# lh3/ropebwt2

Hardware: AMD Instinct MI355X
Metric: Gsymbols/s inserted (wall-clock), bit-identical .fmd (higher is better)
Workload: dtype u8; 1 GPU; configs[1]: 100000000 x 101 bp synthetic reads (splitmix64 seed 42), -bsR -m4g, 1 x MI355X; step = one -m batch (40844297/40844297/18311406 reads); 20 steps = 7 job(s) of 3 batches, each job on an empty index (the last job stops after batch 2); reads_per_job=100000000, symbols=69532236588, symbols_per_gpu=69532236588, parallelism=1 GPU, driver=single engine, counts_ok=True

## Files before the change

include/rb2_hip.h:

```cpp
#ifndef RB2_HIP_H_
#define RB2_HIP_H_

#include <stdint.h>

#ifdef __cplusplus
extern "C" {
#endif

typedef struct rb2_hip_s rb2_hip_t;

#define RB2_SO_IO   0
#define RB2_SO_RLO  1
#define RB2_SO_RCLO 2

typedef void (*rb2_hip_fatal_cb)(void *user, const char *message);
void rb2_hip_set_fatal_handler(rb2_hip_fatal_cb cb, void *user);

int rb2_hip_device_count(void);

rb2_hip_t *rb2_hip_create(int device, int sorting_order);
void rb2_hip_destroy(rb2_hip_t *h);
int  rb2_hip_sorting_order(const rb2_hip_t *h);
void rb2_hip_reset(rb2_hip_t *h);

// ... 71 lines not shown
void  rb2_hip_dev_free(rb2_hip_t *h, void *p);

void rb2_hip_synth_reads(rb2_hip_t *h, uint8_t *dst_dev, int64_t first_read, int64_t n_reads,
                         int read_len, uint64_t seed, int strand);
void rb2_hip_synth_reads_cov(rb2_hip_t *h, uint8_t *dst_dev, int64_t first_read, int64_t n_reads,
                             int read_len, uint64_t seed, int strand, int64_t genome_len);
void rb2_hip_synth_reads_skew(rb2_hip_t *h, uint8_t *dst_dev, int64_t first_read, int64_t n_reads,
                              int read_len, uint64_t seed, int strand, int64_t genome_len, int skew);

void rb2_hip_sync(rb2_hip_t *h);

void rb2_hip_sparse_stats(rb2_hip_t *h, int64_t out[4]);
void rb2_hip_layout_stats(rb2_hip_t *h, int64_t out[8]);
void rb2_hip_rewind_stats(rb2_hip_t *h, int64_t out[4]);
void rb2_hip_window_stats(rb2_hip_t *h, int64_t out[6]);

#define RB2_K_SYM      0
#define RB2_K_TSCAN    1
#define RB2_K_PREP     2
#define RB2_K_PART     3
#define RB2_K_MERGE    4
#define RB2_K_META     5
#define RB2_K_ADVANCE  6
#define RB2_K_INIT     7
#define RB2_K_RELAYOUT 8
#define RB2_K_SPLIT    9
#define RB2_K_COUNT    10
void rb2_hip_profile(rb2_hip_t *h, int enable);
void rb2_hip_profile_get(rb2_hip_t *h, int64_t launches[RB2_K_COUNT], double ms[RB2_K_COUNT],
                         int64_t units[RB2_K_COUNT], int reset);
// ... 9 lines not shown
```

ropebwt2_amd/csrc/rb2_device.h:

```cpp
#pragma once
#include <hip/hip_runtime.h>
#include <stddef.h>
#include <stdint.h>

namespace rb2 {

constexpr int SBITS  = 3;
constexpr int GSYM   = 64;
constexpr int LEAFG  = 16;
constexpr int LEAFW  = SBITS * LEAFG;
constexpr int LEAF   = GSYM * LEAFG;
constexpr int LEAF_SH = 10;
constexpr int SB     = 32;
constexpr int LEAFB  = LEAFW * 8;
#ifndef RB2_GPL
#define RB2_GPL 1
#endif
constexpr int GPL    = RB2_GPL;
constexpr int WPL    = 64 * GPL / LEAFG;
constexpr int WIN    = WPL * LEAF;
constexpr int STILE  = 512;
constexpr int MW     = 4;
constexpr int SCHUNK = 1024;
constexpr int ZBLOCK = 16384;
// ... 46 lines not shown
	uint64_t n0;
	uint64_t len;
	uint32_t ne[2];
	uint32_t wstride;
	uint32_t overflow;
	uint32_t sbfull;
	uint32_t nsplit2[2];
	uint64_t nsplit_total;
	RopeDesc relay_old[NR];
	uint32_t own[NR + 1];
	uint64_t sdest[NR][6];
	uint64_t pdst[NR][6];
	uint32_t pdev[NR][6];
	uint32_t wcnt[16 * 32];
	unsigned long long wfmt[4];
};
constexpr int GCN = NR * 6 + 2;
constexpr int WLC = 16;
constexpr int WLS = 32;

constexpr int NE_RING = 32;
struct Mailbox {
	volatile uint32_t void_round;
	volatile uint32_t respread;
	volatile uint32_t progress;
	uint32_t pad0;
	volatile unsigned long long hmax;
	uint64_t pad1;
	volatile unsigned long long hne;
	uint64_t pad2[3];
	volatile uint32_t ne[NE_RING][2];
// ... 415 lines not shown
```

ropebwt2_amd/csrc/rb2_engine.hip:

```cpp
#include <hip/hip_runtime.h>
#include <cstdio>
#include <cstdlib>
#include <cstring>
#include <climits>
#include <vector>
#include <algorithm>
#include <chrono>
#include <mutex>
#include <thread>
#include <condition_variable>
#include "rb2_hip.h"
#include "rb2_kernels.h"
#include "rb2_query.h"

using namespace rb2;

static rb2_hip_fatal_cb g_fatal_cb = nullptr;
static void *g_fatal_user = nullptr;
#include <cstdarg>
#include <atomic>
#include <mutex>
struct RankFail { std::atomic<int> failed{0}; std::mutex mu; char msg[1024]; };
static thread_local RankFail *t_rank_fail = nullptr;
struct RankAbort {};
// ... 170 lines not shown
	DevBuf<uint64_t> L[2], U[2], W[2], START, SIZE, INS_E, zblk;
	bool pos32 = false, want_pos32 = false;
	int pos_mode = getenv("RB2_POS") ? atoi(getenv("RB2_POS")) : 0;
	uint64_t pos_m0 = 0;
	DevBuf<uint16_t> RKREL;
	DevBuf<uint64_t> RKOLD;
	DevBuf<uint32_t> SPL;
	uint32_t split_epoch = 0;
	bool want_respread = false;
	int64_t n_respread = 0;
	DevBuf<uint64_t> qbuf;
	DevBuf<QTab> qtab;
	DevBuf<uint8_t> qbytes; DevBuf<int64_t> qin, qout;
	uint64_t sp_nsb = 0;
	DevBuf<LeafDesc> LD;
	DevBuf<uint8_t> A[2], INS_A, sbuf;
	DevBuf<uint8_t> sbuf2; hipStream_t st_copy = nullptr; const uint8_t *pf_host = nullptr; size_t pf_done = 0; std::mutex pf_mu;
	bool pf_busy = false; std::condition_variable pf_cv;
	static constexpr int UP_T = 6, UP_NB = 2; static constexpr size_t UP_CH = 8u << 20;
	uint8_t *up_pin[UP_T][UP_NB] = {}; hipStream_t up_st[UP_T] = {}; hipEvent_t up_ev[UP_T][UP_NB] = {}; bool up_init = false;
	DevBuf<TileRec> trec; DevBuf<TileScan> tsc; DevBuf<TileFix> tfix; DevBuf<ChunkPart> cpart;
	DevBuf<SbTot> sbtot;
	uint64_t *d_tmp = nullptr;
	int prof = 0;
	std::vector<ProfRec> recs;
	std::vector<hipEvent_t> evpool;
	int64_t p_launch[RB2_K_COUNT]; double p_ms[RB2_K_COUNT]; int64_t p_units[RB2_K_COUNT];
	int debug = 0;
	int cur_round = -1;
	uint64_t *gcnt = nullptr;
// ... 144 lines not shown
		h->START.ensure(m + 1);
		hipLaunchKernelGGL(k_write_starts, dim3(nzb), dim3(256), 0, st, s, len, h->zblk.p, h->START.p);
	}
	ensure_strings(h, m);
	B.nst_ub = cdiv(m, STILE) + NR;
	B.nsc = cdiv(B.nst_ub, SCHUNK);
	uint64_t n_tot = 0;
	for (int b = 0; b < NR; ++b) n_tot += h->h_rope[b].n;
	const uint64_t leaves_ub = (n_tot + len) / LEAF + NR * (SB + 1);
	if (!h->sparse) {
		h->pool[h->pside].ensure(leaves_ub, true, st);
		h->pool[h->pside ^ 1].ensure(leaves_ub, false, st);
	}
	if (!h->sparse) h->sbtot.ensure(leaves_ub / SB + 1);
	h->LD.ensure(std::max<uint64_t>(leaves_ub + NR + 16, m + 64 + (uint64_t)(NR + WLC + 1) * STILE / 2));
	B.s = s; B.len = len; B.m = m; B.n_tot = n_tot; B.nsb_ub = leaves_ub / SB + 1; B.cur = 0;
	{ uint64_t n0 = 0; for (int b = 0; b < NR; ++b) n0 += h->h_rope[b].cnt[0]; B.known_ae = B.known_ae0 = !is_srt || n0 == 0; }
	{
		uint64_t mx = 0;
		for (int b = 0; b < NR; ++b) mx = std::max<uint64_t>(mx, h->h_rope[b].n);
		h->pos_m0 = mx;
		h->pos32 = h->want_pos32 && h->pos_mode != 64 && mx + 2 * m < POS32_LIMIT;
		h->want_pos32 = false;
		h->mb_h->hmax = 0;
		h->mb_h->progress = 0;
	}
	{
		Scope sc(h, RB2_K_INIT, 0);
		hipLaunchKernelGGL(k_batch_setup, dim3(1), dim3(1), 0, st, h->ctl, h->side, m, len, is_srt);
		with_pos(h, B, [&](const auto &S) { using P = std::remove_pointer_t<decltype(S.L)>;
// ... 58 lines not shown
	hipStream_t st = h->st;
	const int sd = h->side;
	const int64_t units = (int64_t)B.m;
	h->cur_round = (int)r;
	const TileRecs trs = { (uint32_t*)h->trec.p, (uint32_t)(h->trec.cap & ~(size_t)3) };
	tl_slow(h, "start of round_counts");
	const bool one_launch_tail = B.nst_ub < (unsigned)h->ts_max;
	if (!spec) require_verdicts_seen(h, r, "counting phase without spec of round");
	SplitArgs sp; memset(&sp, 0, sizeof(sp));
	if (spec) {
	  sp.ctl = h->ctl; sp.pool = h->pool[h->pside].view(); sp.SPL = h->SPL.p; sp.spl_cap = split_cap(h); sp.epoch = h->split_epoch;
	  sp.mb = h->mb_d; sp.nsplitb = 64;
	  sp.round1 = (uint32_t)r;
	  sp.scan2 = (h->dir_ride && !one_launch_tail) ? sp.pool.sbbase : (SbBase*)nullptr;
	}
	SbBase *scan2_tail = (spec && h->dir_ride && one_launch_tail) ? h->pool[h->pside].view().sbbase : (SbBase*)nullptr;
	{ Scope sc(h, RB2_K_SYM, units);
	  with_pos(h, B, [&](const auto &S) { using P = std::remove_pointer_t<decltype(S.L)>;
	    if (spec) {
	      hipLaunchKernelGGL((k_sym<false, P, true>), dim3((unsigned)rank_share(h, B.nst_ub) + sp.nsplitb + (sp.scan2 ? 1u : 0u)), dim3(256), 0, st, h->ctl, sd, (int)(r & 1), S, trs, sp);
	    } else
	    RB2_LAUNCH_STRIDE(h, (k_sym<true, P>), (k_sym<false, P>), dim3(grid8((unsigned)rank_share(h, B.nst_ub))), dim3(256), 0, st, h->ctl, sd, (int)(r & 1), S, trs, sp); }); }
	tl_slow(h, "k_sym");
	if (spec && !lazy_round(h, spec)) HIPCHK(hipEventRecord(h->ev_flag, st));
	if (one_launch_tail) {
	  Scope sc(h, RB2_K_TSCAN, units);
	  const int do_setup = h->nranks == 1;
	  const unsigned grid = (unsigned)std::max(1, std::min<int>(TSB, h->ts_blocks)) + (scan2_tail ? 7u : 0u);
	  hipLaunchKernelGGL((h->sparse ? k_tscan_setup<true> : k_tscan_setup<false>), dim3(grid), dim3(SCHUNK), 0, st, h->ctl, sd, (int)(r & 1), trs, h->tfix.p, h->gcnt, do_setup, (int)spec, (uint32_t)r, hmax_report(h), scan2_tail);
	  if (do_setup) mark_setup(h, B, r);
	} else
	{ Scope sc(h, RB2_K_TSCAN, units);
	  hipLaunchKernelGGL(k_tscan1, dim3(B.nsc), dim3(SCHUNK), 0, st, h->ctl, sd, trs, h->cpart.p);
	  if (B.nsc <= (unsigned)h->ts_fold) hipLaunchKernelGGL(k_tscan3<true>, dim3(B.nsc), dim3(SCHUNK), 0, st, h->ctl, sd, trs, h->cpart.p, h->tsc.p);
	  else {
	    hipLaunchKernelGGL(k_tscan2, dim3(1), dim3(SCHUNK), 0, st, h->ctl, sd, h->cpart.p);
	    hipLaunchKernelGGL(k_tscan3<false>, dim3(B.nsc), dim3(SCHUNK), 0, st, h->ctl, sd, trs, h->cpart.p, h->tsc.p);
// ... 28 lines not shown
	hipStream_t st = h->st;
	const int sd = h->side;
	const int64_t units = (int64_t)B.m;
	PoolView oldp = h->pool[h->pside].view(), newp = h->pool[h->pside ^ 1].view();
	const uint64_t n_new_ub = B.n_tot + std::min<uint64_t>(B.len, (r + 1) * B.m);
	const unsigned nlf = cdiv(n_new_ub, WIN) + NR;
	const unsigned wg = cdiv(B.n_tot + rank_share(h, std::min<uint64_t>(B.len, (r + 1) * B.m)), WIN) + NR;
	if ((uint64_t)nlf * 64 >= (1ull << 32)) { rb2_fatal("[rb2_hip] the index is too large for one k_merge launch (%llu symbols: a launch is capped at 2^32 threads)\n", (unsigned long long)n_new_ub); }
	if (!setup_done(h, B, r, false))
	{ Scope sc(h, RB2_K_TSCAN, 0);
	  hipLaunchKernelGGL(k_setup<false>, dim3(1), dim3(64), 0, st, h->ctl, sd, h->gcnt, (int)(r & 1), (uint32_t)r, hmax_report(h), (int)(h->push[0] != nullptr)); }
	with_pos(h, B, [&](const auto &S) { using P = std::remove_pointer_t<decltype(S.L)>;
	launch_prep<false>(h, B, r, oldp, S);
	tl_slow(h, "k_prep");
	{ Scope sc(h, RB2_K_PART, units);
	  RB2_LAUNCH_STRIDE(h, (k_part<true, P>), (k_part<false, P>), dim3(cdiv(wg + NR, 255)), dim3(256), 0, st, h->ctl, sd, S.INS_E, h->LD.p, h->pool_compact ? (const uint8_t*)oldp.xh : (const uint8_t*)nullptr); }
	tl_slow(h, "k_part");
	{ Scope sc(h, RB2_K_MERGE, units);
	  RB2_LAUNCH_STRIDE(h, (k_merge<true, P>), (k_merge<false, P>), dim3(grid8(cdiv(wg, MMW))), dim3(64 * MMW), 0, st, h->ctl, h->LD.p, oldp, newp, S.INS_E, S.INS_A, S.RKREL, (int)compact_out | (h->compact_stats ? 2 : 0), (int)(r & 1)); }
	tl_slow(h, "k_merge");
	{ Scope sc(h, RB2_K_META, units);
	  build_directory(h, sd ^ 1, h->pside ^ 1, std::min<uint64_t>(B.nsb_ub, n_new_ub / (LEAF * SB) + NR + 1), false, false, (uint64_t)wg * WPL / SB + NR + 1); }
	tl_slow(h, "directory");
	launch_advance<false>(h, B, r, newp, S, send, ScanRide{ nullptr, 0u });
	});
	tl_slow(h, "k_advance");
	if (!B.known_ae && !send && h->nranks == 1) ne_snapshot(h, r);
	HIPCHK(hipGetLastError());
	tl_slow(h, "ne snapshot");
	h->side ^= 1; h->pside ^= 1; B.cur ^= 1;
	h->pool_compact = compact_out;
// ... 329 lines not shown
	if (getenv("RB2_SPARSE_MAXPEN")) h->sp_maxpen = atoi(getenv("RB2_SPARSE_MAXPEN"));
	if (h->trace) h->prof = 1;
	HIPCHK(hipStreamCreateWithFlags(&h->st, hipStreamNonBlocking));
	HIPCHK(hipMalloc((void**)&h->ctl, sizeof(Ctl)));
	HIPCHK(hipMalloc((void**)&h->d_tmp, 256));
	HIPCHK(hipMalloc((void**)&h->gcnt, GCN * 8));
	HIPCHK(hipHostMalloc((void**)&h->mb_h, sizeof(Mailbox), hipHostMallocDefault));
	memset(h->mb_h, 0, sizeof(Mailbox));
	HIPCHK(hipHostGetDevicePointer((void**)&h->mb_d, h->mb_h, 0));
	HIPCHK(hipEventCreateWithFlags(&h->ev_flag, hipEventDisableTiming));
	if (getenv("RB2_DIR_RIDE")) h->dir_ride = atoi(getenv("RB2_DIR_RIDE"));
	if (getenv("RB2_TS_BLOCKS")) h->ts_blocks = atoi(getenv("RB2_TS_BLOCKS"));
	if (getenv("RB2_LAZY_VERDICT")) h->lazy_verdict = atoi(getenv("RB2_LAZY_VERDICT"));
	if (getenv("RB2_RUN_AHEAD")) h->run_ahead = std::max(1, atoi(getenv("RB2_RUN_AHEAD")));
	if (getenv("RB2_VERDICT_POLL")) h->verdict_poll = atoi(getenv("RB2_VERDICT_POLL"));
	{ Ctl *hc = (Ctl*)calloc(1, sizeof(Ctl)); for (int b = 0; b < NR; ++b) hc->own[b] = 1; HIPCHK(hipMemcpy(h->ctl, hc, sizeof(Ctl), hipMemcpyHostToDevice)); free(hc); }
	HIPCHK(hipMemsetAsync(h->d_tmp, 0, 256, h->st));
	memset(h->h_rope, 0, sizeof(h->h_rope));
	memset(h->p_launch, 0, sizeof(h->p_launch)); memset(h->p_ms, 0, sizeof(h->p_ms)); memset(h->p_units, 0, sizeof(h->p_units));
	h->pool[0].ensure(SB * 8, false, h->st); h->pool[1].ensure(SB * 8, false, h->st);
	HIPCHK(hipStreamSynchronize(h->st));
	return h;
}

void rb2_hip_destroy(rb2_hip_t *h)
{ finish_pending(h);
	if (!h) return;
	HIPCHK(hipSetDevice(h->dev));
	if (h->own_stream) HIPCHK(hipStreamSynchronize(h->st)); else HIPCHK(hipDeviceSynchronize());
	for (int i = 0; i < 2; ++i) { h->pool[i].release(); h->L[i].release(); h->U[i].release(); h->W[i].release(); }
	h->START.release(); h->SIZE.release(); h->INS_E.release(); h->RKREL.release(); h->RKOLD.release(); h->SPL.release(); h->qbuf.release(); h->zblk.release(); h->qtab.release(); h->qbytes.release(); h->qin.release(); h->qout.release();
	h->LD.release(); h->A[0].release(); h->A[1].release(); h->INS_A.release(); h->sbuf.release(); h->sbuf2.release();
	if (h->st_copy) HIPCHK(hipStreamDestroy(h->st_copy));
	h->trec.release(); h->tsc.release(); h->tfix.release(); h->cpart.release(); h->sbtot.release();
	for (auto e : h->evpool) hipEventDestroy(e);
	HIPCHK(hipHostFree(h->mb_h)); HIPCHK(hipEventDestroy(h->ev_flag));

	if (h->pair_d) { HIPCHK(hipFree(h->pair_d)); HIPCHK(hipHostFree(h->pair_h)); }
	HIPCHK(hipFree(h->ctl)); HIPCHK(hipFree(h->d_tmp)); HIPCHK(hipFree(h->gcnt)); h->xstage.release(); h->xnb.release(); h->xpack.release(); h->xoff.release();
	for (int i = 0; i < 2; ++i) if (h->xhost[i]) { HIPCHK(hipHostFree(h->xhost[i])); HIPCHK(hipHostFree(h->xtot[i])); HIPCHK(hipEventDestroy(h->xev[i])); }
	if (h->own_stream) HIPCHK(hipStreamDestroy(h->st));
	delete h;
}

int rb2_hip_sorting_order(const rb2_hip_t *h) { return h->so; }

void rb2_hip_reset(rb2_hip_t *h)
// ... 543 lines not shown
	rb2_hip_synth_reads_cov(h, dst_dev, first_read, n_reads, read_len, seed, strand, 0);
}

void rb2_hip_reserve(rb2_hip_t *h, int64_t batch_bytes, int64_t batch_strings, int64_t total_symbols)
{ finish_pending(h);
	HIPCHK(hipSetDevice(h->dev));
	if (batch_bytes > 0) h->zblk.ensure(cdiv((uint64_t)batch_bytes, ZBLOCK) + 2);
	if (batch_strings > 0) ensure_strings(h, (uint64_t)batch_strings);
	if (total_symbols > 0) {
		const uint64_t leaves = (uint64_t)total_symbols / LEAF + NR * (SB + 1);
		size_t fr = 0, tot = 0;
		if (hipMemGetInfo(&fr, &tot) == hipSuccess && 2.0 * leaves * (LEAFB + 2.0 * sizeof(LeafMeta) + 2.0) > 0.6 * (double)fr) return;
		h->pool[h->pside].ensure(leaves, true, h->st);
		h->pool[h->pside ^ 1].ensure(leaves, false, h->st);
		h->LD.ensure(leaves + NR + 16);
		if (!h->sparse) h->sbtot.ensure(leaves / SB + 1);
	}
}

void rb2_hip_sparse_stats(rb2_hip_t *h, int64_t out[4])
{ finish_pending(h);
	out[0] = h->n_relayout; out[1] = h->n_void; out[2] = h->n_sparse_rounds; out[3] = h->sparse ? 1 : 0;
}

void rb2_hip_layout_stats(rb2_hip_t *h, int64_t out[8])
{ finish_pending(h);
	uint64_t ns = 0;
	HIPCHK(hipSetDevice(h->dev));
	HIPCHK(hipMemcpyAsync(&ns, &h->ctl->nsplit_total, 8, hipMemcpyDeviceToHost, h->st));
	HIPCHK(hipStreamSynchronize(h->st));
// ... 4 lines not shown
void rb2_hip_rewind_stats(rb2_hip_t *h, int64_t out[4])
{ finish_pending(h);
	out[0] = h->n_rewind; out[1] = h->n_rewound; out[2] = h->rewind_max; out[3] = h->n_rewind_even;
}

void rb2_hip_window_stats(rb2_hip_t *h, int64_t out[6])
{ finish_pending(h);
	unsigned long long w[4] = {0, 0, 0, 0};
	HIPCHK(hipSetDevice(h->dev));
	HIPCHK(hipMemcpyAsync(w, &h->ctl->wfmt[0], sizeof(w), hipMemcpyDeviceToHost, h->st));
	HIPCHK(hipStreamSynchronize(h->st));
	for (int i = 0; i < 4; ++i) out[i] = (int64_t)w[i];
	out[4] = h->n_compact_rounds; out[5] = h->compact_stats ? 1 : 0;
}

void rb2_hip_sync(rb2_hip_t *h) { finish_pending(h); HIPCHK(hipSetDevice(h->dev)); HIPCHK(hipStreamSynchronize(h->st)); }

void rb2_hip_profile(rb2_hip_t *h, int enable) { finish_pending(h); h->prof = enable; }

void rb2_hip_profile_get(rb2_hip_t *h, int64_t launches[RB2_K_COUNT], double ms[RB2_K_COUNT], int64_t units[RB2_K_COUNT], int reset)
{ finish_pending(h);
	for (int k = 0; k < RB2_K_COUNT; ++k) { launches[k] = h->p_launch[k]; ms[k] = h->p_ms[k]; units[k] = h->p_units[k]; }
	if (reset) { memset(h->p_launch, 0, sizeof(h->p_launch)); memset(h->p_ms, 0, sizeof(h->p_ms)); memset(h->p_units, 0, sizeof(h->p_units)); }
}

const char *rb2_hip_kernel_name(int k)
{
	static const char *nm[RB2_K_COUNT] = {"k_sym", "k_tscan", "k_prep", "k_part", "k_merge", "k_meta", "k_advance", "k_init", "k_relayout", "k_split"};
	return (k >= 0 && k < RB2_K_COUNT) ? nm[k] : "?";
}
// ... 12 lines not shown
```

ropebwt2_amd/csrc/rb2_kernels.h:

```cpp
#pragma once
#include "rb2_device.h"

namespace rb2 {


__device__ __forceinline__ uint32_t zero_bytes(uint32_t x)
{
	const uint32_t t = ((x & 0x7f7f7f7fu) + 0x7f7f7f7fu) | x;
	return __popc(~t & 0x80808080u);
}

__device__ __forceinline__ void load64(const uint8_t *s, uint64_t len, uint64_t base, uint32_t w[16])
{
	if (base + 64 <= len) {
		const uint4 *p = (const uint4*)(s + base);
#pragma unroll
		for (int i = 0; i < 4; ++i) { uint4 v = p[i]; w[4*i] = v.x; w[4*i+1] = v.y; w[4*i+2] = v.z; w[4*i+3] = v.w; }
	} else {
#pragma unroll
		for (int i = 0; i < 16; ++i) {
			uint32_t x = 0;
			for (int k = 0; k < 4; ++k) {
				const uint64_t p = base + 4*i + k;
				x |= (uint32_t)(p < len ? s[p] : 0xffu) << (8*k);
// ... 162 lines not shown
__global__ __launch_bounds__(256) void k_widen(const uint32_t *src, uint64_t *dst, uint64_t n)
{
	const uint64_t i = (uint64_t)blockIdx.x * 256 + threadIdx.x;
	if (i < n) dst[i] = src[i];
}

__global__ void k_batch_setup(Ctl *ctl, int side, uint64_t m, uint64_t len, int is_srt)
{
	if (threadIdx.x || blockIdx.x) return;
	SegDesc &sg = ctl->seg[side];
	for (int b = 0; b < NR; ++b) { sg.start[b] = 0; sg.cnt[b] = 0; }
	sg.cnt[0] = ctl->own[0] ? m : 0;
	uint32_t t = 0;
	for (int b = 0; b < NR; ++b) { sg.tile0[b] = t; t += (uint32_t)((sg.cnt[b] + STILE - 1) / STILE); }
	sg.tile0[NR] = t; sg.tile0[NR + 1] = t;
	uint64_t n0 = 0;
	for (int b = 0; b < NR; ++b) n0 += ctl->rope[side][b].cnt[0];
	ctl->n0 = n0; ctl->n_strings = m; ctl->max_len = 0; ctl->len = len;
	ctl->ne[0] = (is_srt && n0) ? 1u : 0u;
	ctl->ne[1] = 0;
}


struct TileCtx { int b; uint64_t lt, base, segstart, segend; };

__device__ __forceinline__ bool tile_ctx(const SegDesc &sg, uint32_t tile, TileCtx &t)
{
	if (tile >= sg.tile0[NR]) return false;
	const int b = seg_of(sg.tile0, tile);
	t.b = b; t.lt = tile - sg.tile0[b];
	t.segstart = sg.start[b]; t.segend = sg.start[b] + sg.cnt[b];
	t.base = t.segstart + t.lt * STILE;
	return true;
}

struct SplitArgs { Ctl *ctl; PoolView pool; const uint32_t *SPL; uint32_t spl_cap, epoch; Mailbox *mb; uint32_t nsplitb;
	uint32_t round1;
	SbBase *scan2; };
template <int NT, int CT> __device__ __forceinline__ void sbscan2_lean(const Ctl *ctl, SbBase *base, uint64_t *s_w );
template <int NT, int CT> __device__ __forceinline__ void sbscan2_col(const Ctl *ctl, SbBase *base, uint64_t *s_w, const int col);
__device__ __forceinline__ void split_body(Ctl *ctl, const PoolView &pool, const uint32_t *SPL, uint32_t spl_cap, uint32_t epoch, Mailbox *mb,
		const uint32_t bidx, const uint32_t nblk, uint16_t (*s_row)[7][SB], uint32_t round1);
constexpr int32_t TILE_DONE = 0x10000;
constexpr int32_t TILE_SINGLE = 0x20000;
template <bool STRIDE, typename P = uint64_t, bool SPLIT = false> __global__ __launch_bounds__(256) void k_sym(const Ctl *ctl, int side, int par, StrArrays<P> S, TileRecs trec, SplitArgs sp)
{
	const P *L = S.L, *UU = S.U; P *INS_E = S.INS_E; uint8_t *INS_A = S.INS_A, *A = S.A;
	__shared__ uint64_t s_bal[8][6], s_head[8];
	__shared__ __align__(16) uint32_t s_ok[4];
	if (SPLIT) {
		__shared__ uint16_t s_row[MW][7][SB];
		if (blockIdx.x < sp.nsplitb) { split_body(sp.ctl, sp.pool, sp.SPL, sp.spl_cap, sp.epoch, sp.mb, blockIdx.x, sp.nsplitb, s_row, sp.round1); return; }
		if (sp.scan2 && blockIdx.x == sp.nsplitb) { __shared__ uint64_t s_w2[4]; sbscan2_lean<256, 2>(ctl, sp.scan2, s_w2); return; }
	}
	const bool ae = ctl->ne[par] == 0;
	const P *U = ae ? L : UU;
	for (uint32_t tile = (STRIDE || SPLIT) ? blockIdx.x - (SPLIT ? sp.nsplitb + (sp.scan2 ? 1u : 0u) : 0u) : xcd_item(); ; tile += gridDim.x) {
	if (STRIDE && tile != blockIdx.x) __syncthreads();
	TileCtx t;
	if (!tile_ctx(ctl->seg[side], tile, t)) return;
	const int ln = lane_id(), w = wave_id();
	const uint32_t nval = (uint32_t)min((uint64_t)STILE, t.segend - t.base);
	const uint8_t *Ab = A + t.base; const P *Ub = U + t.base;
	const bool first_tile = t.base == t.segstart;
	uint32_t av[2]; P uv[2], up[2], un = 0;
#pragma unroll
	for (int h = 0; h < 2; ++h) {
		const uint32_t x = (uint32_t)(h * 256) + threadIdx.x;
		RB2_UNDEFV(av[h]); RB2_UNDEFV(uv[h]); RB2_UNDEFV(up[h]);
		if (x < nval) { av[h] = Ab[x]; uv[h] = Ub[x]; up[h] = (x > 0 || !first_tile) ? Ub[(int32_t)x - 1] : (P)0; }
	}
	const bool last_thread = threadIdx.x == 255;
	const bool has_next = last_thread && t.base + STILE < t.segend;
	if (has_next) un = Ub[STILE];
	bool single = true;
	int sym2[2];
	uint8_t *Aw = A + t.base;
#pragma unroll
	for (int h = 0; h < 2; ++h) {
		const uint32_t x = (uint32_t)(h * 256) + threadIdx.x;
		int sym = 7; bool head = false;
		if (x < nval) {
			sym = (int)(av[h] & 7);
			head = (x == 0 && first_tile) || (uv[h] != up[h]);
			Aw[x] = (uint8_t)(sym | (head ? 0x80 : 0));
			single = single && head;
		}
		sym2[h] = sym;
		const int c = h * 4 + w;
// ... 11 lines not shown
	{ const uint64_t sm = ballot64(single); if (ln == 0) s_ok[w] = sm == ~0ull ? 1u : 0u; }
	__syncthreads();
	const uint4 okv = *(const uint4*)s_ok;
	const bool allsingle = (okv.x & okv.y & okv.z & okv.w) != 0;
	const bool fused = ae && allsingle;
	if (fused) {
		P *Eb = INS_E + t.base; uint8_t *Ib = INS_A + t.base;
		const P slot0 = (P)(t.lt * STILE);
#pragma unroll
		for (int h = 0; h < 2; ++h) {
			const uint32_t x = (uint32_t)(h * 256) + threadIdx.x;
			if (x >= nval) continue;
			Eb[x] = (P)(uv[h] - (slot0 + (P)x));
			Ib[x] = (uint8_t)sym2[h];
		}
	}
	if (threadIdx.x < 6) {
		const int s = threadIdx.x;
		uint32_t run = 0, fhpre = 0, lhpre = 0; int fh = -1, lh = -1;
		if (allsingle) {
#pragma unroll
			for (int c = 0; c < 8; ++c) run += __popcll(s_bal[c][s]);
			if (nval) { fh = 0; lh = (int)nval - 1; lhpre = run - (uint32_t)((s_bal[lh >> 6][s] >> (lh & 63)) & 1ull); }
		} else
		for (int c = 0; c < 8; ++c) {
			const uint64_t hm = s_head[c], bm = s_bal[c][s];
			if (hm) {
				const int f = __builtin_ctzll(hm), l = 63 - __builtin_clzll(hm);
				if (fh < 0) { fh = c * 64 + f; fhpre = run + __popcll(bm & lt_mask(f)); }
				lh = c * 64 + l; lhpre = run + __popcll(bm & lt_mask(l));
			}
// ... 193 lines not shown
		const uint64_t pinc = dpp_incl_add64(padded), winc = dpp_incl_add64(nwin);
		n.leaf0 = pinc - padded; n.sb0 = n.leaf0 / SB;
		if (ok) { ctl->rope[side ^ 1][r] = n; ctl->wf0[r] = winc - nwin; }
		if (r == 63) { ctl->wf0[NR] = winc; ctl->wf0[NR + 1] = winc; ctl->nsb_total = pinc / SB; }
	}
	uint64_t c2 = 0;
	if (ok && r != 0 && ctl->own[r]) {
		const int a = rope_sym(r), b = rope_prev(r);
		if (b == 0) c2 = gcnt[a];
		else for (int x = 0; x < 6; ++x) c2 += gcnt[rope_of(b, x) * 6 + a];
	}
	const uint64_t cinc = dpp_incl_add64(c2), st = cinc - c2;
	const uint32_t nt = (uint32_t)((c2 + STILE - 1) / STILE);
	const uint32_t tinc = dpp_incl_add(nt);
	if (ok) { ng.start[r] = st; ng.cnt[r] = c2; ng.tile0[r] = tinc - nt; }
	if (r == 63) { ng.tile0[NR] = tinc; ng.tile0[NR + 1] = tinc; }
	for (int a = 1; a < 6; ++a) {
		const int r2 = rope_of(a, rope_sym(rr));
		const uint64_t st2 = __shfl(st, r2);
		uint64_t before = 0;
		if (rope_sym(rr) != 0) for (int x = 0; x < rope_prev(rr); ++x) before += gcnt[rope_of(rope_sym(rr), x) * 6 + a];
		if (ok) ctl->dest[r][a] = st2 + before;
	}
	if (ok) ctl->dest[r][0] = 0;
}
template <bool SPARSE> __global__ __launch_bounds__(64) void k_setup(Ctl *ctl, int side, const uint64_t *gcnt, int par, uint32_t round, volatile unsigned long long *hmax, int keep_ne)
{
	if (blockIdx.x) return;
	setup_body<SPARSE>(ctl, side, gcnt, par, round, hmax, keep_ne != 0);
}
// ... 336 lines not shown
			prep_tile<AE, SPARSE, P>(t0 + k, ctl, side, par, is_comp, oldp, S);
			if (todo) __syncthreads();
		}
		return;
	}
	for (uint32_t tile = STRIDE ? blockIdx.x : xcd_item(); ; ) {
		if (!prep_tile<AE, SPARSE, P>(tile, ctl, side, par, is_comp, oldp, S)) return;
		if (!STRIDE) return;
		tile += gridDim.x;
		if (tile >= ctl->seg[side].tile0[NR]) return;
		__syncthreads();
	}
}


template <bool STRIDE, typename P = uint64_t> __global__ __launch_bounds__(256) void k_part(const Ctl *ctl, int side, const P *INS_E, LeafDesc *LD, const uint8_t *old_xh)
{
	__shared__ uint64_t s_wf0[NR + 1];
	__shared__ uint32_t s_q[256];
	if (threadIdx.x <= NR) s_wf0[threadIdx.x] = ctl->wf0[threadIdx.x];
	__syncthreads();
	for (uint64_t blk = blockIdx.x; blk * 255 < s_wf0[NR] + NR; blk += gridDim.x) {
	if (STRIDE && blk != blockIdx.x) __syncthreads();
	const uint64_t gid = blk * 255 + threadIdx.x;
	const bool ok = gid < s_wf0[NR] + NR;
	int b = 0; uint64_t j = 0; uint32_t q = 0;
	if (ok) {
		while (gid >= s_wf0[b+1] + b + 1) ++b;
		j = gid - s_wf0[b] - b;
		const SegDesc &sg = ctl->seg[side];
		const P *E = INS_E + sg.start[b];
		const uint64_t o = j * WIN;
		uint64_t lo = 0, hi = sg.cnt[b];
		while (lo < hi) {
			const uint64_t mid = (lo + hi) >> 1;
			if (E[mid] + mid >= o) hi = mid; else lo = mid + 1;
		}
		q = (uint32_t)lo;
	}
	s_q[threadIdx.x] = q;
	__syncthreads();
	if (!ok || threadIdx.x == 255 || j >= s_wf0[b+1] - s_wf0[b]) { if (!STRIDE) return; continue; }
	const RopeDesc &orp = ctl->rope[side][b], &nrp = ctl->rope[side ^ 1][b];
	const uint32_t q1 = s_q[threadIdx.x + 1];
	const uint64_t o0 = j * WIN, i0 = o0 - q;
	LeafDesc d;
	d.i0 = i0;
	d.ins0 = ctl->seg[side].start[b] + q;
	d.gl = nrp.leaf0 + j * WPL;
	d.oleaf0 = (uint32_t)orp.leaf0;
	const uint64_t ow = i0 >> 12, onw = (orp.nleaves + WPL - 1) / WPL;
	static_assert(WPL * LEAF == 4096, "a window is 4096 symbols");
	const uint8_t *xw = old_xh ? old_xh + orp.leaf0 / WPL : nullptr;
	const uint32_t h0 = ow < onw ? (xw ? (uint32_t)xw[ow] & 3u : 0u) : 1u;
	const uint32_t h1 = ow + 1 < onw ? (xw ? (uint32_t)xw[ow + 1] & 3u : 0u) : 1u;
	d.ni = (uint16_t)((uint32_t)(q1 - q) | h0 << 14);
	d.nvalid = (uint16_t)((uint32_t)min((uint64_t)WIN, nrp.n - o0) | h1 << 14);
	LD[s_wf0[b] + j] = d;
	if (!STRIDE) return;
// ... 972 lines not shown
```

ropebwt2_amd/hipbwt.py:

```python
import ctypes as C
import os

import numpy as np

from .build import lib_path

K_NAMES = ["k_sym", "k_tscan", "k_prep", "k_part", "k_merge", "k_meta", "k_advance", "k_init", "k_relayout", "k_split"]
_lib = None


def load_hip_lib():
    global _lib
    if _lib is not None:
        return _lib
    path = os.environ.get("RB2_HIP_LIB") or lib_path("librb2hip.so")
    if not os.path.exists(path):
        raise RuntimeError("%s missing: run `python -m ropebwt2_amd.build` (hipcc, gfx950) first" % path)
    L = C.CDLL(path)
    vp, i64, i32, u64 = C.c_void_p, C.c_int64, C.c_int, C.c_uint64
    sig = {
        "rb2_hip_device_count": (i32, []),
        "rb2_hip_set_fatal_handler": (None, [vp, vp]),
        "rb2_hip_create": (vp, [i32, i32]),
        "rb2_hip_destroy": (None, [vp]),
# ... 19 lines not shown
        "rb2_hip_extract": (i64, [vp, i64, vp, i64, vp, vp]),
        "rb2_hip_reserve": (None, [vp, i64, i64, i64]),
        "rb2_hip_num_subropes": (i32, []),
        "rb2_hip_memcpy": (None, [vp, vp, vp, i64, i32]),
        "rb2_hip_use_stream": (None, [vp, vp]),
        "rb2_hip_dev_alloc": (vp, [vp, i64]),
        "rb2_hip_dev_free": (None, [vp, vp]),
        "rb2_hip_synth_reads": (None, [vp, vp, i64, i64, i32, u64, i32]),
        "rb2_hip_synth_reads_cov": (None, [vp, vp, i64, i64, i32, u64, i32, i64]),
        "rb2_hip_synth_reads_skew": (None, [vp, vp, i64, i64, i32, u64, i32, i64, i32]),
        "rb2_hip_sync": (None, [vp]),
        "rb2_hip_sparse_stats": (None, [vp, vp]),
        "rb2_hip_layout_stats": (None, [vp, vp]),
        "rb2_hip_rewind_stats": (None, [vp, vp]),
        "rb2_hip_window_stats": (None, [vp, vp]),
        "rb2_hip_host_register": (C.c_int, [vp, C.c_int64]),
        "rb2_hip_host_unregister": (C.c_int, [vp]),
        "rb2_hip_profile": (None, [vp, i32]),
        "rb2_hip_profile_get": (None, [vp, vp, vp, vp, i32]),
        "rb2_hip_kernel_name": (C.c_char_p, [i32]),
        "rb2_hip_layout": (None, [vp, vp, vp]),
        "rb2_hip_multi_create": (vp, [i32, vp, i32, i32, vp]),
        "rb2_hip_multi_unique_id": (None, [vp]),
        "rb2_hip_multi_create_rank": (vp, [i32, i32, i32, vp, i32, vp]),
        "rb2_hip_multi_destroy": (None, [vp]),
        "rb2_hip_default_owners": (None, [i32, vp]),
        "rb2_hip_multi_nranks": (i32, [vp]),
        "rb2_hip_multi_transport": (i32, [vp]),
        "rb2_hip_multi_nlocal": (i32, [vp]),
        "rb2_hip_multi_engine": (vp, [vp, i32]),
# ... 21 lines not shown
            if os.environ.get("RB2_HIP_LIB"):
                continue
            raise
        f.restype = res
        f.argtypes = args
    _lib = L
    return L


ABI_SYMBOLS = [
    "rb2_hip_device_count", "rb2_hip_set_fatal_handler", "rb2_hip_create", "rb2_hip_destroy", "rb2_hip_sorting_order", "rb2_hip_reset",
    "rb2_hip_insert_multi", "rb2_hip_insert_multi_dev", "rb2_hip_set_lazy", "rb2_hip_wait", "rb2_hip_last_batch_counts", "rb2_hip_prefetch", "rb2_hip_mem_info", "rb2_hip_get_counts", "rb2_hip_rope_bytes",
    "rb2_hip_download_rope", "rb2_hip_stream_rope", "rb2_hip_load_ropes", "rb2_hip_rank1a", "rb2_hip_rank_batch", "rb2_hip_reserve",
    "rb2_hip_backward_search", "rb2_hip_backward_search_dev", "rb2_hip_extend", "rb2_hip_extract", "rb2_hip_dev_alloc",
    "rb2_hip_num_subropes", "rb2_hip_memcpy", "rb2_hip_use_stream",
    "rb2_hip_dev_free", "rb2_hip_synth_reads", "rb2_hip_synth_reads_cov", "rb2_hip_synth_reads_skew", "rb2_hip_sync", "rb2_hip_sparse_stats", "rb2_hip_layout_stats", "rb2_hip_rewind_stats", "rb2_hip_window_stats", "rb2_hip_host_register", "rb2_hip_host_unregister", "rb2_hip_profile",
    "rb2_hip_profile_get", "rb2_hip_kernel_name", "rb2_hip_layout",
    "rb2_hip_multi_create", "rb2_hip_multi_unique_id", "rb2_hip_multi_create_rank", "rb2_hip_multi_destroy", "rb2_hip_default_owners",
    "rb2_hip_multi_nranks", "rb2_hip_multi_transport", "rb2_hip_multi_nlocal", "rb2_hip_multi_engine", "rb2_hip_multi_insert_multi", "rb2_hip_multi_insert_multi_dev",
    "rb2_hip_multi_get_counts", "rb2_hip_multi_rope_bytes", "rb2_hip_multi_download_rope", "rb2_hip_multi_stream_rope",
    "rb2_hip_multi_load_ropes", "rb2_hip_multi_reserve", "rb2_hip_multi_rope_hash", "rb2_hip_rope_hash", "rb2_hip_multi_plan_host", "rb2_hip_multi_reset", "rb2_hip_multi_sync", "rb2_hip_multi_rank1a", "rb2_hip_multi_stats", "rb2_hip_multi_text_bytes",
]


_NT6 = np.full(256, 255, dtype=np.uint8)
for _i, _ch in enumerate("$ACGTN"):
    _NT6[ord(_ch)] = _NT6[ord(_ch.lower())] = _i


def encode_pattern(p):
    if isinstance(p, str):
# ... 192 lines not shown
        a = np.zeros(8, np.int64)
        self.L.rb2_hip_layout_stats(self.h, a.ctypes.data)
        return {"relayouts": int(a[0]), "void_rounds": int(a[1]), "sparse_rounds": int(a[2]), "sparse_now": bool(a[3]),
                "respreads": int(a[4]), "leaf_splits": int(a[5]), "grown_in_rounds": int(a[6]), "plain_handovers": int(a[7])}

    def rewind_stats(self):
        a = np.zeros(4, np.int64)
        self.L.rb2_hip_rewind_stats(self.h, a.ctypes.data)
        return {"rewinds": int(a[0]), "rounds_taken_back": int(a[1]), "deepest": int(a[2]), "even_depth": int(a[3])}

    def window_stats(self):
        a = np.zeros(6, np.int64)
        self.L.rb2_hip_window_stats(self.h, a.ctypes.data)
        return {"plain": int(a[0]), "compact0": int(a[1]), "compact1": int(a[2]), "compact2": int(a[3]), "compact_rounds": int(a[4]), "counted": bool(a[5])}

    def profile(self, on=True):
        self.L.rb2_hip_profile(self.h, int(on))

    def profile_get(self, reset=False):
        n = len(K_NAMES)
        la = np.zeros(n, np.int64)
        ms = np.zeros(n, np.float64)
        un = np.zeros(n, np.int64)
        self.L.rb2_hip_profile_get(self.h, la.ctypes.data, ms.ctypes.data, un.ctypes.data, 1 if reset else 0)
        return {K_NAMES[i]: {"launches": int(la[i]), "ms": float(ms[i]), "units": int(un[i])} for i in range(n)}

    @staticmethod
    def layout():
        L = load_hip_lib()
        a, b, c = C.c_int(), C.c_int(), C.c_int()
# ... 116 lines not shown
```

Baseline: 23.10 Gsymbols/s.

## Build window-to-insert lookup table in k_sym so k_part skips binary search

k_sym now scatters, for each insertion, its index into a per-window table QT, using per-rope window offsets that are precomputed in the segment setup and advance kernels. k_part then reads the window start indices straight from this table and no longer binary-searches INS_E per window, which also removes a shared-memory exchange and a barrier. The change adds scattered writes in k_sym, extra Ctl fields and a fallback flag (q_bad) that returns k_part to the binary search when runs are too long or the capacity is exceeded. A verify mode (2) counts mismatches for debugging.

```diff
diff --git a/include/rb2_hip.h b/include/rb2_hip.h
--- a/include/rb2_hip.h
+++ b/include/rb2_hip.h
@@ -109,6 +109,7 @@
 void rb2_hip_layout_stats(rb2_hip_t *h, int64_t out[8]);
 void rb2_hip_rewind_stats(rb2_hip_t *h, int64_t out[4]);
 void rb2_hip_window_stats(rb2_hip_t *h, int64_t out[6]);
+void rb2_hip_part_table_stats(rb2_hip_t *h, int64_t out[4]);
 
 #define RB2_K_SYM      0
 #define RB2_K_TSCAN    1
diff --git a/ropebwt2_amd/csrc/rb2_device.h b/ropebwt2_amd/csrc/rb2_device.h
--- a/ropebwt2_amd/csrc/rb2_device.h
+++ b/ropebwt2_amd/csrc/rb2_device.h
@@ -84,7 +84,13 @@
 	uint32_t pdev[NR][6];
 	uint32_t wcnt[16 * 32];
 	unsigned long long wfmt[4];
-};
+	uint32_t q_bad;
+	uint32_t q_rounds;
+	uint32_t q_mismatch;
+	uint32_t q_pad;
+	uint64_t q_wf0[2][NR + 1];
+};
+struct QArgs { uint32_t *Q; uint32_t cap, run, pad; };
 constexpr int GCN = NR * 6 + 2;
 constexpr int WLC = 16;
 constexpr int WLS = 32;
diff --git a/ropebwt2_amd/csrc/rb2_engine.hip b/ropebwt2_amd/csrc/rb2_engine.hip
--- a/ropebwt2_amd/csrc/rb2_engine.hip
+++ b/ropebwt2_amd/csrc/rb2_engine.hip
@@ -208,6 +208,9 @@
 	DevBuf<uint8_t> qbytes; DevBuf<int64_t> qin, qout;
 	uint64_t sp_nsb = 0;
 	DevBuf<LeafDesc> LD;
+	DevBuf<uint32_t> QT;
+	int part_table = 1;
+	uint32_t q_run = 0;
 	DevBuf<uint8_t> A[2], INS_A, sbuf;
 	DevBuf<uint8_t> sbuf2; hipStream_t st_copy = nullptr; const uint8_t *pf_host = nullptr; size_t pf_done = 0; std::mutex pf_mu;
 	bool pf_busy = false; std::condition_variable pf_cv;
@@ -382,6 +385,7 @@
 	}
 	if (!h->sparse) h->sbtot.ensure(leaves_ub / SB + 1);
 	h->LD.ensure(std::max<uint64_t>(leaves_ub + NR + 16, m + 64 + (uint64_t)(NR + WLC + 1) * STILE / 2));
+	if (h->nranks == 1 && h->part_table) h->QT.ensure(leaves_ub / WPL + NR + 16);
 	B.s = s; B.len = len; B.m = m; B.n_tot = n_tot; B.nsb_ub = leaves_ub / SB + 1; B.cur = 0;
 	{ uint64_t n0 = 0; for (int b = 0; b < NR; ++b) n0 += h->h_rope[b].cnt[0]; B.known_ae = B.known_ae0 = !is_srt || n0 == 0; }
 	{
@@ -470,13 +474,15 @@
 	  sp.round1 = (uint32_t)r;
 	  sp.scan2 = (h->dir_ride && !one_launch_tail) ? sp.pool.sbbase : (SbBase*)nullptr;
 	}
+	if (++h->q_run == 0) h->q_run = 1;
+	const QArgs qa = { (h->nranks == 1 && h->part_table) ? h->QT.p : (uint32_t*)nullptr, (uint32_t)std::min<size_t>(h->QT.cap, 0xffffffffu), h->q_run, 0u };
 	SbBase *scan2_tail = (spec && h->dir_ride && one_launch_tail) ? h->pool[h->pside].view().sbbase : (SbBase*)nullptr;
 	{ Scope sc(h, RB2_K_SYM, units);
 	  with_pos(h, B, [&](const auto &S) { using P = std::remove_pointer_t<decltype(S.L)>;
 	    if (spec) {
-	      hipLaunchKernelGGL((k_sym<false, P, true>), dim3((unsigned)rank_share(h, B.nst_ub) + sp.nsplitb + (sp.scan2 ? 1u : 0u)), dim3(256), 0, st, h->ctl, sd, (int)(r & 1), S, trs, sp);
+	      hipLaunchKernelGGL((k_sym<false, P, true>), dim3((unsigned)rank_share(h, B.nst_ub) + sp.nsplitb + (sp.scan2 ? 1u : 0u)), dim3(256), 0, st, h->ctl, sd, (int)(r & 1), S, trs, sp, qa);
 	    } else
-	    RB2_LAUNCH_STRIDE(h, (k_sym<true, P>), (k_sym<false, P>), dim3(grid8((unsigned)rank_share(h, B.nst_ub))), dim3(256), 0, st, h->ctl, sd, (int)(r & 1), S, trs, sp); }); }
+	    RB2_LAUNCH_STRIDE(h, (k_sym<true, P>), (k_sym<false, P>), dim3(grid8((unsigned)rank_share(h, B.nst_ub))), dim3(256), 0, st, h->ctl, sd, (int)(r & 1), S, trs, sp, qa); }); }
 	tl_slow(h, "k_sym");
 	if (spec && !lazy_round(h, spec)) HIPCHK(hipEventRecord(h->ev_flag, st));
 	if (one_launch_tail) {
@@ -535,7 +541,8 @@
 	launch_prep<false>(h, B, r, oldp, S);
 	tl_slow(h, "k_prep");
 	{ Scope sc(h, RB2_K_PART, units);
-	  RB2_LAUNCH_STRIDE(h, (k_part<true, P>), (k_part<false, P>), dim3(cdiv(wg + NR, 255)), dim3(256), 0, st, h->ctl, sd, S.INS_E, h->LD.p, h->pool_compact ? (const uint8_t*)oldp.xh : (const uint8_t*)nullptr); }
+	  RB2_LAUNCH_STRIDE(h, (k_part<true, P>), (k_part<false, P>), dim3(cdiv(wg + NR, 255)), dim3(256), 0, st, h->ctl, sd, S.INS_E, h->LD.p, h->pool_compact ? (const uint8_t*)oldp.xh : (const uint8_t*)nullptr,
+	    (const uint32_t*)h->QT.p, (uint32_t)std::min<size_t>(h->QT.cap, 0xffffffffu), h->q_run, h->nranks == 1 ? h->part_table : 0, (int)(r & 1)); }
 	tl_slow(h, "k_part");
 	{ Scope sc(h, RB2_K_MERGE, units);
 	  RB2_LAUNCH_STRIDE(h, (k_merge<true, P>), (k_merge<false, P>), dim3(grid8(cdiv(wg, MMW))), dim3(64 * MMW), 0, st, h->ctl, h->LD.p, oldp, newp, S.INS_E, S.INS_A, S.RKREL, (int)compact_out | (h->compact_stats ? 2 : 0), (int)(r & 1)); }
@@ -895,6 +902,7 @@
 	if (getenv("RB2_LAZY_VERDICT")) h->lazy_verdict = atoi(getenv("RB2_LAZY_VERDICT"));
 	if (getenv("RB2_RUN_AHEAD")) h->run_ahead = std::max(1, atoi(getenv("RB2_RUN_AHEAD")));
 	if (getenv("RB2_VERDICT_POLL")) h->verdict_poll = atoi(getenv("RB2_VERDICT_POLL"));
+	if (getenv("RB2_PART_TABLE")) h->part_table = std::max(0, std::min(2, atoi(getenv("RB2_PART_TABLE"))));
 	{ Ctl *hc = (Ctl*)calloc(1, sizeof(Ctl)); for (int b = 0; b < NR; ++b) hc->own[b] = 1; HIPCHK(hipMemcpy(h->ctl, hc, sizeof(Ctl), hipMemcpyHostToDevice)); free(hc); }
 	HIPCHK(hipMemsetAsync(h->d_tmp, 0, 256, h->st));
 	memset(h->h_rope, 0, sizeof(h->h_rope));
@@ -911,7 +919,7 @@
 	if (h->own_stream) HIPCHK(hipStreamSynchronize(h->st)); else HIPCHK(hipDeviceSynchronize());
 	for (int i = 0; i < 2; ++i) { h->pool[i].release(); h->L[i].release(); h->U[i].release(); h->W[i].release(); }
 	h->START.release(); h->SIZE.release(); h->INS_E.release(); h->RKREL.release(); h->RKOLD.release(); h->SPL.release(); h->qbuf.release(); h->zblk.release(); h->qtab.release(); h->qbytes.release(); h->qin.release(); h->qout.release();
-	h->LD.release(); h->A[0].release(); h->A[1].release(); h->INS_A.release(); h->sbuf.release(); h->sbuf2.release();
+	h->LD.release(); h->QT.release(); h->A[0].release(); h->A[1].release(); h->INS_A.release(); h->sbuf.release(); h->sbuf2.release();
 	if (h->st_copy) HIPCHK(hipStreamDestroy(h->st_copy));
 	h->trec.release(); h->tsc.release(); h->tfix.release(); h->cpart.release(); h->sbtot.release();
 	for (auto e : h->evpool) hipEventDestroy(e);
@@ -1485,6 +1493,7 @@
 		h->pool[h->pside].ensure(leaves, true, h->st);
 		h->pool[h->pside ^ 1].ensure(leaves, false, h->st);
 		h->LD.ensure(leaves + NR + 16);
+		if (h->nranks == 1 && h->part_table) h->QT.ensure(leaves / WPL + NR + 16);
 		if (!h->sparse) h->sbtot.ensure(leaves / SB + 1);
 	}
 }
@@ -1519,6 +1528,15 @@
 	out[4] = h->n_compact_rounds; out[5] = h->compact_stats ? 1 : 0;
 }
 
+void rb2_hip_part_table_stats(rb2_hip_t *h, int64_t out[4])
+{ finish_pending(h);
+	uint32_t w[4] = {0, 0, 0, 0};
+	HIPCHK(hipSetDevice(h->dev));
+	HIPCHK(hipMemcpyAsync(w, &h->ctl->q_bad, sizeof(w), hipMemcpyDeviceToHost, h->st));
+	HIPCHK(hipStreamSynchronize(h->st));
+	out[0] = (int64_t)w[1]; out[1] = (int64_t)w[2]; out[2] = h->part_table; out[3] = 0;
+}
+
 void rb2_hip_sync(rb2_hip_t *h) { finish_pending(h); HIPCHK(hipSetDevice(h->dev)); HIPCHK(hipStreamSynchronize(h->st)); }
 
 void rb2_hip_profile(rb2_hip_t *h, int enable) { finish_pending(h); h->prof = enable; }
diff --git a/ropebwt2_amd/csrc/rb2_kernels.h b/ropebwt2_amd/csrc/rb2_kernels.h
--- a/ropebwt2_amd/csrc/rb2_kernels.h
+++ b/ropebwt2_amd/csrc/rb2_kernels.h
@@ -200,6 +200,8 @@
 	uint32_t t = 0;
 	for (int b = 0; b < NR; ++b) { sg.tile0[b] = t; t += (uint32_t)((sg.cnt[b] + STILE - 1) / STILE); }
 	sg.tile0[NR] = t; sg.tile0[NR + 1] = t;
+	{ uint32_t w0 = 0;
+	  for (int b = 0; b < NR; ++b) { const uint32_t nw = (uint32_t)((ctl->rope[side][b].n + sg.cnt[b] + (uint64_t)(WIN - 1)) / (uint64_t)WIN); ctl->q_wf0[0][b] = (uint64_t)(w0 + (uint32_t)b) | (uint64_t)nw << 32; w0 += nw; } }
 	uint64_t n0 = 0;
 	for (int b = 0; b < NR; ++b) n0 += ctl->rope[side][b].cnt[0];
 	ctl->n0 = n0; ctl->n_strings = m; ctl->max_len = 0; ctl->len = len;
@@ -229,7 +231,8 @@
 		const uint32_t bidx, const uint32_t nblk, uint16_t (*s_row)[7][SB], uint32_t round1);
 constexpr int32_t TILE_DONE = 0x10000;
 constexpr int32_t TILE_SINGLE = 0x20000;
-template <bool STRIDE, typename P = uint64_t, bool SPLIT = false> __global__ __launch_bounds__(256) void k_sym(const Ctl *ctl, int side, int par, StrArrays<P> S, TileRecs trec, SplitArgs sp)
+constexpr uint32_t QRUN_MAX = 1024;
+template <bool STRIDE, typename P = uint64_t, bool SPLIT = false> __global__ __launch_bounds__(256) void k_sym(const Ctl *ctl, int side, int par, StrArrays<P> S, TileRecs trec, SplitArgs sp, QArgs qa)
 {
 	const P *L = S.L, *UU = S.U; P *INS_E = S.INS_E; uint8_t *INS_A = S.INS_A, *A = S.A;
 	__shared__ uint64_t s_bal[8][6], s_head[8];
@@ -241,6 +244,7 @@
 	}
 	const bool ae = ctl->ne[par] == 0;
 	const P *U = ae ? L : UU;
+	const bool qon = !STRIDE && qa.Q != nullptr;
 	for (uint32_t tile = (STRIDE || SPLIT) ? blockIdx.x - (SPLIT ? sp.nsplitb + (sp.scan2 ? 1u : 0u) : 0u) : xcd_item(); ; tile += gridDim.x) {
 	if (STRIDE && tile != blockIdx.x) __syncthreads();
 	TileCtx t;
@@ -259,6 +263,8 @@
 	const bool last_thread = threadIdx.x == 255;
 	const bool has_next = last_thread && t.base + STILE < t.segend;
 	if (has_next) un = Ub[STILE];
+	uint64_t qw = 0;
+	if (qon) qw = ctl->q_wf0[par][t.b];
 	bool single = true;
 	int sym2[2];
 	uint8_t *Aw = A + t.base;
@@ -300,7 +306,31 @@
 			Eb[x] = (P)(uv[h] - (slot0 + (P)x));
 			Ib[x] = (uint8_t)sym2[h];
 		}
-	}
+		if (qon) {
+			const uint32_t qb = (uint32_t)qw, nwb = (uint32_t)(qw >> 32);
+			uint32_t *Qb = qa.Q + qb;
+			const uint32_t room = qb < qa.cap ? qa.cap - qb : 0u;
+			bool bad = false;
+			auto fill = [&](uint32_t j0, uint32_t j1, uint32_t v) {
+				if (j1 > room) { bad = true; return; }
+				if (j1 <= j0) return;
+				if (j1 - j0 > QRUN_MAX) { bad = true; return; }
+				for (uint32_t j = j0; j < j1; ++j) Qb[j] = v;
+			};
+#pragma unroll
+			for (int h = 0; h < 2; ++h) {
+				const uint32_t x = (uint32_t)(h * 256) + threadIdx.x;
+				if (x >= nval) continue;
+				const uint32_t q = (uint32_t)slot0 + x;
+				const uint32_t wq = (uint32_t)min((uint64_t)uv[h] >> 12, (uint64_t)nwb);
+				const uint32_t j0 = (x == 0 && first_tile) ? 0u : (uint32_t)min((uint64_t)up[h] >> 12, (uint64_t)nwb) + 1u;
+				fill(j0, wq + 1u, q);
+				if (t.base + x + 1 == t.segend) fill(wq + 1u, nwb + 1u, q + 1u);
+			}
+			if (bad) const_cast<Ctl*>(ctl)->q_bad = qa.run;
+		}
+	}
+	else if (qon && threadIdx.x == 0 && (ae || tile == 0)) const_cast<Ctl*>(ctl)->q_bad = qa.run;
 	if (threadIdx.x < 6) {
 		const int s = threadIdx.x;
 		uint32_t run = 0, fhpre = 0, lhpre = 0; int fh = -1, lh = -1;
@@ -524,6 +554,11 @@
 	const uint32_t nt = (uint32_t)((c2 + STILE - 1) / STILE);
 	const uint32_t tinc = dpp_incl_add(nt);
 	if (ok) { ng.start[r] = st; ng.cnt[r] = c2; ng.tile0[r] = tinc - nt; }
+	{
+		const uint32_t nwn = ok ? (uint32_t)((n.n + c2 + (uint64_t)(WIN - 1)) / (uint64_t)WIN) : 0u;
+		const uint32_t wn = dpp_incl_add(nwn);
+		if (ok) ctl->q_wf0[(round + 1u) & 1u][r] = (uint64_t)(wn - nwn + (uint32_t)r) | (uint64_t)nwn << 32;
+	}
 	if (r == 63) { ng.tile0[NR] = tinc; ng.tile0[NR + 1] = tinc; }
 	for (int a = 1; a < 6; ++a) {
 		const int r2 = rope_of(a, rope_sym(rr));
@@ -890,35 +925,53 @@
 }
 
 
-template <bool STRIDE, typename P = uint64_t> __global__ __launch_bounds__(256) void k_part(const Ctl *ctl, int side, const P *INS_E, LeafDesc *LD, const uint8_t *old_xh)
+template <bool STRIDE, typename P = uint64_t> __global__ __launch_bounds__(256) void k_part(const Ctl *ctl, int side, const P *INS_E, LeafDesc *LD, const uint8_t *old_xh,
+		const uint32_t *Q, uint32_t qcap, uint32_t qrun, int qmode, int qpar)
 {
 	__shared__ uint64_t s_wf0[NR + 1];
 	__shared__ uint32_t s_q[256];
 	if (threadIdx.x <= NR) s_wf0[threadIdx.x] = ctl->wf0[threadIdx.x];
-	__syncthreads();
+	const bool tab = !STRIDE && qmode != 0 && Q != nullptr && ctl->q_bad != qrun && ctl->wf0[NR] + NR <= (uint64_t)qcap;
+	const bool fast = tab && qmode != 2;
+	__syncthreads();
+	if (tab && blockIdx.x == 0) {
+		Ctl *wctl = const_cast<Ctl*>(ctl);
+		if (threadIdx.x == 0) atomicAdd(&wctl->q_rounds, 1u);
+		if (qmode == 2 && threadIdx.x < NR) {
+			const int b = threadIdx.x;
+			if (ctl->q_wf0[qpar][b] != ((s_wf0[b] + b) | (s_wf0[b + 1] - s_wf0[b]) << 32)) atomicAdd(&wctl->q_mismatch, 1u);
+		}
+	}
 	for (uint64_t blk = blockIdx.x; blk * 255 < s_wf0[NR] + NR; blk += gridDim.x) {
 	if (STRIDE && blk != blockIdx.x) __syncthreads();
 	const uint64_t gid = blk * 255 + threadIdx.x;
 	const bool ok = gid < s_wf0[NR] + NR;
-	int b = 0; uint64_t j = 0; uint32_t q = 0;
+	int b = 0; uint64_t j = 0; uint32_t q = 0, q1 = 0;
 	if (ok) {
 		while (gid >= s_wf0[b+1] + b + 1) ++b;
 		j = gid - s_wf0[b] - b;
 		const SegDesc &sg = ctl->seg[side];
-		const P *E = INS_E + sg.start[b];
-		const uint64_t o = j * WIN;
-		uint64_t lo = 0, hi = sg.cnt[b];
-		while (lo < hi) {
-			const uint64_t mid = (lo + hi) >> 1;
-			if (E[mid] + mid >= o) hi = mid; else lo = mid + 1;
-		}
-		q = (uint32_t)lo;
-	}
-	s_q[threadIdx.x] = q;
-	__syncthreads();
+		if (fast) {
+			if (sg.cnt[b] != 0) { q = Q[gid]; if (j < s_wf0[b+1] - s_wf0[b]) q1 = Q[gid + 1]; }
+		} else {
+			const P *E = INS_E + sg.start[b];
+			const uint64_t o = j * WIN;
+			uint64_t lo = 0, hi = sg.cnt[b];
+			while (lo < hi) {
+				const uint64_t mid = (lo + hi) >> 1;
+				if (E[mid] + mid >= o) hi = mid; else lo = mid + 1;
+			}
+			q = (uint32_t)lo;
+			if (tab && threadIdx.x != 255 && (sg.cnt[b] != 0 ? Q[gid] : 0u) != q) atomicAdd(&const_cast<Ctl*>(ctl)->q_mismatch, 1u);
+		}
+	}
+	if (!fast) {
+		s_q[threadIdx.x] = q;
+		__syncthreads();
+	}
 	if (!ok || threadIdx.x == 255 || j >= s_wf0[b+1] - s_wf0[b]) { if (!STRIDE) return; continue; }
 	const RopeDesc &orp = ctl->rope[side][b], &nrp = ctl->rope[side ^ 1][b];
-	const uint32_t q1 = s_q[threadIdx.x + 1];
+	if (!fast) q1 = s_q[threadIdx.x + 1];
 	const uint64_t o0 = j * WIN, i0 = o0 - q;
 	LeafDesc d;
 	d.i0 = i0;
diff --git a/ropebwt2_amd/hipbwt.py b/ropebwt2_amd/hipbwt.py
--- a/ropebwt2_amd/hipbwt.py
+++ b/ropebwt2_amd/hipbwt.py
@@ -57,6 +57,7 @@
         "rb2_hip_layout_stats": (None, [vp, vp]),
         "rb2_hip_rewind_stats": (None, [vp, vp]),
         "rb2_hip_window_stats": (None, [vp, vp]),
+        "rb2_hip_part_table_stats": (None, [vp, vp]),
         "rb2_hip_host_register": (C.c_int, [vp, C.c_int64]),
         "rb2_hip_host_unregister": (C.c_int, [vp]),
         "rb2_hip_profile": (None, [vp, i32]),
@@ -108,7 +109,7 @@
     "rb2_hip_download_rope", "rb2_hip_stream_rope", "rb2_hip_load_ropes", "rb2_hip_rank1a", "rb2_hip_rank_batch", "rb2_hip_reserve",
     "rb2_hip_backward_search", "rb2_hip_backward_search_dev", "rb2_hip_extend", "rb2_hip_extract", "rb2_hip_dev_alloc",
     "rb2_hip_num_subropes", "rb2_hip_memcpy", "rb2_hip_use_stream",
-    "rb2_hip_dev_free", "rb2_hip_synth_reads", "rb2_hip_synth_reads_cov", "rb2_hip_synth_reads_skew", "rb2_hip_sync", "rb2_hip_sparse_stats", "rb2_hip_layout_stats", "rb2_hip_rewind_stats", "rb2_hip_window_stats", "rb2_hip_host_register", "rb2_hip_host_unregister", "rb2_hip_profile",
+    "rb2_hip_dev_free", "rb2_hip_synth_reads", "rb2_hip_synth_reads_cov", "rb2_hip_synth_reads_skew", "rb2_hip_sync", "rb2_hip_sparse_stats", "rb2_hip_layout_stats", "rb2_hip_rewind_stats", "rb2_hip_window_stats", "rb2_hip_part_table_stats", "rb2_hip_host_register", "rb2_hip_host_unregister", "rb2_hip_profile",
     "rb2_hip_profile_get", "rb2_hip_kernel_name", "rb2_hip_layout",
     "rb2_hip_multi_create", "rb2_hip_multi_unique_id", "rb2_hip_multi_create_rank", "rb2_hip_multi_destroy", "rb2_hip_default_owners",
     "rb2_hip_multi_nranks", "rb2_hip_multi_transport", "rb2_hip_multi_nlocal", "rb2_hip_multi_engine", "rb2_hip_multi_insert_multi", "rb2_hip_multi_insert_multi_dev",
@@ -331,6 +332,11 @@
         self.L.rb2_hip_window_stats(self.h, a.ctypes.data)
         return {"plain": int(a[0]), "compact0": int(a[1]), "compact1": int(a[2]), "compact2": int(a[3]), "compact_rounds": int(a[4]), "counted": bool(a[5])}
 
+    def part_table_stats(self):
+        a = np.zeros(4, np.int64)
+        self.L.rb2_hip_part_table_stats(self.h, a.ctypes.data)
+        return {"table_rounds": int(a[0]), "mismatches": int(a[1]), "mode": int(a[2])}
+
     def profile(self, on=True):
         self.L.rb2_hip_profile(self.h, int(on))
 
```

After: 23.02 Gsymbols/s. Within noise of the previous version (-0.4%).
